# sayands/sgaligner

Measured on AMD Instinct MI355X. Metric: subscan-pairs/sec (fwd+bwd) + node-match Hits@1 vs reference, higher is better.
Workload: dtype f32 (fp32 operands and fp32 accumulation throughout; the anchors x negatives loss sweeps multiply them as three exact bf16 planes, six bf16 MFMAs per product...

## Files before the change

sgaligner_amd/csrc/sweep3.hip:

```cpp
#include <type_traits>

#include "loss_math.h"
#include "s3_layout.h"

namespace {

__device__ __forceinline__ void split3_pair(float v0, float v1, unsigned& h, unsigned& m, unsigned& l) {
    const bf16x2 H = __builtin_convertvector(f32x2{v0, v1}, bf16x2);
    const unsigned hu = __builtin_bit_cast(unsigned, H);
#ifdef S3_SPLIT_DOT2
    unsigned c0 = 0x0000BF80u, c1 = 0xBF800000u;
    asm("" : "+s"(c0), "+s"(c1));
    const bf16x2 n0 = __builtin_bit_cast(bf16x2, c0), n1 = __builtin_bit_cast(bf16x2, c1);
    const float r0 = __builtin_amdgcn_fdot2_f32_bf16(H, n0, v0, false);
    const float r1 = __builtin_amdgcn_fdot2_f32_bf16(H, n1, v1, false);
#else
    const float r0 = v0 - __builtin_bit_cast(float, hu << 16);
    const float r1 = v1 - __builtin_bit_cast(float, hu & 0xffff0000u);
#endif
    const bf16x2 Mi = __builtin_convertvector(f32x2{r0, r1}, bf16x2);
    const unsigned mu = __builtin_bit_cast(unsigned, Mi);
#ifdef S3_SPLIT_DOT2
    const float s0 = __builtin_amdgcn_fdot2_f32_bf16(Mi, n0, r0, false);
    const float s1 = __builtin_amdgcn_fdot2_f32_bf16(Mi, n1, r1, false);
// ... 74 lines not shown
    __syncthreads();
    if (threadIdx.x < 32) {
        const int r = threadIdx.x;
        if (r < nvalid) {
            double a = 0.0;
            for (int c = 0; c < S3_DREAL; ++c) a += (double)zbar[c] * (double)tile[r * S3_DP + c];
            tile[r * S3_DP + S3_DREAL] = (float)(a + (double)stat[S3_DP]);
            tile[r * S3_DP + S3_DREAL + 1] = 1.f;
        }
    }
    __syncthreads();
    unsigned* out = reinterpret_cast<unsigned*>(Zb + (size_t)blockIdx.x * S3_BLOCK);
    for (int e = threadIdx.x; e < 3 * 2 * 64 * 4; e += 256) {
        const int p = e & 3, st = (e >> 2) & 63, jh = (e >> 8) & 1, q = e >> 9;
        const int g = st >> 4, i = (st & 15) ^ (12 * (g & 1));
        const int row = 8 * (i >> 2) + 4 * jh + (i & 3), col = 32 * q + 8 * g + 2 * p;
        unsigned h, m, l;
        split3_pair(tile[row * S3_DP + col], tile[row * S3_DP + col + 1], h, m, l);
        out[e] = h; out[S3_PLANE / 4 + e] = m; out[2 * S3_PLANE / 4 + e] = l;
    }
    for (int e = threadIdx.x; e < 2 * 64 * 4; e += 256) {
        const int p = e & 3, st = (e >> 2) & 63, jh = (e >> 8) & 1;
        const int g = st >> 4, i = (st & 15) ^ (12 * (g & 1));
        const int row = 8 * (i >> 2) + 4 * jh + (i & 3), col = 96 + 2 * p;
        unsigned h, m, l;
        split3_pair(tile[row * S3_DP + col], tile[row * S3_DP + col + 1], h, m, l);
        out[S3_TAIL / 4 + e] = g < 2 ? h : (g == 2 ? m : l);
    }
}


__global__ __launch_bounds__(256) void centre_tables_kernel(const float* __restrict__ Z, int R, const float* __restrict__ stat, float* __restrict__ Zc) {
    const int lane = threadIdx.x & 63, wpb = blockDim.x >> 6;
    for (int r = blockIdx.x * wpb + (threadIdx.x >> 6); r < R; r += gridDim.x * wpb) {
        const float* z = Z + (size_t)r * S3_DP;
        float* o = Zc + (size_t)r * S3_DP;
        double acc = 0.0;
        float v[2];
#pragma unroll
        for (int t = 0; t < 2; ++t) {
            const int d = lane + 64 * t;
            const float zb = d < S3_DREAL ? stat[d] : 0.f;
            v[t] = d < S3_DREAL ? z[d] - zb : 0.f;
            acc += (double)zb * (double)v[t];
        }
        acc = wave_sum_d(acc);
        o[lane] = v[0];
        const int d1 = lane + 64;
        if (d1 < S3_DP) o[d1] = d1 < S3_DREAL ? v[1] : (d1 == S3_DREAL ? (float)(acc + (double)stat[S3_DP]) : (d1 == S3_DREAL + 1 ? 1.f : 0.f));
    }
}

#ifdef S3_DBG_TIMING
__device__ unsigned long long g_s3_dbg[16];
#define S3_T(i) { const unsigned long long t_ = __builtin_readcyclecounter(); tacc[i] += t_ - tprev; tprev = t_; }
#else
#define S3_T(i)
#endif
struct TSeg { int blk0, jt_lo, jt_hi, old0, lo, hi, fam; };
struct TGroup { int own0, nown, own_old0, own_blk0, blk0, nsplit, nseg; TSeg seg[2]; };
struct TArgs {
    int M; const unsigned char* Zb[4]; int perm[4]; int ngroups; TGroup grp[4];
    float k0, k1, it0, it1, ka;
    const float* beta;
    double* sums;
    const double* gs;
    float* dZ[4];
    double* gamma;
};

#ifndef S3_PAIR
#define S3_PAIR 1
#endif
template <int M, int PER> struct S3PairGaps {
    int slot[M][40];
    constexpr S3PairGaps() : slot{} {
        for (int p = 0; p < M; ++p) {
            int n = 0;
            for (int P = 0; P < 40; ++P) {
                const bool copy = p < M - 1 && P % (20 / PER) == 1 && P / (20 / PER) < 2 * PER;
                slot[p][P] = (P >= 3 && !copy) ? n++ : -1;
            }
        }
    }
};

template <int M, bool GRAD, int WV, int MG, bool GAM, bool LITE, bool FOLD>
__device__ __forceinline__ void sweep3_body(const TArgs& a, const int g) {
    static_assert(!LITE || !GRAD, "LITE: the forward sums only");
    static_assert(!FOLD || (GRAD && WV == 4), "FOLD: the one-wave-per-SIMD gradient sweep only");
    constexpr int NCT = 7;
    constexpr int WAVES = WV, THREADS = WAVES * 64;
    constexpr int OWN = WV * 16;
    constexpr int NCH = LITE ? S3_NCH - S3_PLANE / 1024 : S3_NCH;
    constexpr int KMAX = (NCH + WAVES - 1) / WAVES;
    constexpr int BUF = M * S3_BLOCK;
    constexpr bool PIPE = WV == 4;
#ifndef S3_OWN_IN_S
#define S3_OWN_IN_S 1
#endif
    constexpr bool OWN_IN_S = GRAD && PIPE && S3_OWN_IN_S;
#ifndef S3_SPREAD
#define S3_SPREAD 1
#endif
    constexpr bool SPREAD = OWN_IN_S && S3_SPREAD && !FOLD;
    constexpr bool PAIR_FITS = !(!GRAD && WV == 8 && M == 3 && !LITE);
    constexpr bool PAIR_DEFAULT = !(GRAD && M == 2) && !(!GRAD && M == 4 && !LITE);
    constexpr bool PAIR = PAIR_FITS && (S3_PAIR == 2 || (S3_PAIR == 1 && PAIR_DEFAULT));
    extern __shared__ __attribute__((aligned(16))) unsigned char lds3[];

    const int tid = threadIdx.x, lane = tid & 63, wave = tid >> 6, g4 = lane >> 4, l15 = lane & 15;
    const TGroup& grp = a.grp[g];
    const int wg_in_grp = (int)blockIdx.x - grp.blk0;
    const int nsplit = grp.nsplit, n_ob = (grp.nown + OWN - 1) / OWN, n_units = n_ob * nsplit;
    const int unit = (wg_in_grp & 7) * ((n_units + 7) >> 3) + (wg_in_grp >> 3);
    if ((wg_in_grp >> 3) >= ((n_units + 7) >> 3) || unit >= n_units) return;
    const int split = unit / n_ob;
    const int own0 = grp.own0 + (unit - split * n_ob) * OWN;
    const int own_end = grp.own0 + grp.nown;
    const int wrow0 = own0 + wave * 16;
#ifdef S3_DBG_TIMING
    unsigned long long tacc[8] = {0, 0, 0, 0, 0, 0, 0, 0}, tprev = __builtin_readcyclecounter();
#endif

    u32x4 opl[M][3][3], otl[M][2];
    float beta[M];
    const bool iv = wrow0 + l15 < own_end;
    {
        const int my_i = wrow0 + l15;
        const int rel = (iv ? my_i : own0) - grp.own_old0;
        const int o = rel & 31, oi = 4 * (o >> 3) + (o & 3), ojh = (o >> 2) & 1;
        const size_t off = (size_t)(grp.own_blk0 + (rel >> 5)) * S3_BLOCK;
#pragma unroll
        for (int m = 0; m < M; ++m) {
            const unsigned char* base = a.Zb[m] + off;
#pragma unroll
            for (int p = 0; p < 3; ++p)
#pragma unroll
                for (int q = 0; q < 3; ++q) {
                    const int so = ((q * 2 + ojh) * 64 + s3_slot(g4, oi)) * 16;
                    opl[m][p][q] = iv ? *reinterpret_cast<const u32x4*>(base + p * S3_PLANE + so) : u32x4{0, 0, 0, 0};
                }
            u32x4 th = iv ? *reinterpret_cast<const u32x4*>(base + S3_TAIL + (ojh * 64 + s3_slot(0, oi)) * 16) : u32x4{0, 0, 0, 0};
            u32x4 tm = iv ? *reinterpret_cast<const u32x4*>(base + S3_TAIL + (ojh * 64 + s3_slot(2, oi)) * 16) : u32x4{0, 0, 0, 0};
            u32x4 tl = iv ? *reinterpret_cast<const u32x4*>(base + S3_TAIL + (ojh * 64 + s3_slot(3, oi)) * 16) : u32x4{0, 0, 0, 0};
            const float ksc = a.k1;
            auto rescale = [&](u32x4& ph, u32x4& pm, u32x4& pl) {
#pragma unroll
                for (int d = 0; d < 4; ++d) {
                    const float x0 = (__builtin_bit_cast(float, ph[d] << 16) + __builtin_bit_cast(float, pm[d] << 16)) + __builtin_bit_cast(float, pl[d] << 16);
                    const float x1 = (__builtin_bit_cast(float, ph[d] & 0xffff0000u) + __builtin_bit_cast(float, pm[d] & 0xffff0000u)) + __builtin_bit_cast(float, pl[d] & 0xffff0000u);
                    unsigned nh, nm, nl;
                    split3_pair(x0 * ksc, x1 * ksc, nh, nm, nl);
                    ph[d] = nh; pm[d] = nm; pl[d] = nl;
                }
            };
#pragma unroll
            for (int q = 0; q < 3; ++q) rescale(opl[m][0][q], opl[m][1][q], opl[m][2][q]);
            rescale(th, tm, tl);
            s3_own_tails(th, tm, tl, g4, otl[m]);
        }
// ... 42 lines not shown
        buf_off = (unsigned)(buf - lds3);
#pragma unroll
        for (int m = 0; m < M; ++m) {
            trot[m] = tile_off + crot[m]; brot[m] = buf_off + (unsigned)(m * S3_BLOCK) + crot[m];
            asm("" : "+s"(trot[m]), "+s"(brot[m]));
        }
    };
    auto issue_slots = [&](int f_lo, int f_hi) {
#ifdef S3_DBG_NODMA
        return;
#endif
#ifdef S3_DBG_DMA_WAVES
        unsigned dma_mask = S3_DBG_DMA_WAVES;
        asm volatile("" : "+s"(dma_mask));
        if (!((dma_mask >> wave_u) & 1u)) return;
#endif
#pragma unroll
        for (int f = f_lo; f < f_hi; ++f) {
            if (f >= M * KMAX) break;
            const int m = f / KMAX, k = f % KMAX;
            unsigned so, lo;
            if (LAST_ODD && k == KMAX - 1) { so = tile_off + clast[m]; lo = buf_off + (unsigned)(m * S3_BLOCK) + clast[m]; }
            else { so = trot[m] + (unsigned)(k * WAVES * 1024); lo = brot[m] + (unsigned)(k * WAVES * 1024); }
            __builtin_amdgcn_raw_ptr_buffer_load_lds(rs[m], (lds_ptr)lds3 + lo, 16, l16, so, 0, 0);
        }
    };
    auto issue = [&](int jt, unsigned char* buf) { set_tile(jt, buf); issue_slots(0, M * KMAX); };

    const int aoff = s3_slot(g4, l15) * 16;
    const int tr_io = 4 * g4 + (l15 >> 2), tr_cs = l15 & 3;
    const int tr_main = s3_slot(tr_cs >> 1, tr_io) * 16 + (tr_cs & 1) * 8;
    const int tr_tail = S3_TAIL + tr_io * 16 + (tr_cs & 1) * 8;
    const int tr_tail_l = S3_TAIL + (48 + (tr_io ^ 12)) * 16 + (tr_cs & 1) * 8;

#pragma unroll 1
    for (int sg = 0; sg < 2; ++sg) {
        if (sg >= grp.nseg) break;
        const TSeg seg = grp.seg[sg];
        set_seg(seg);
        float c0[M + 1], c1[M + 1];
#pragma unroll
        for (int m = 0; m <= M; ++m) {
            const int mo = m < M ? a.perm[m] : M;
            c0[m] = GRAD ? (float)(a.gs[mo * 8 + seg.fam * 2 + 0] * (double)a.it0) : 0.f;
            c1[m] = GRAD ? (float)(a.gs[mo * 8 + seg.fam * 2 + 1] * (double)a.it1) : 0.f;
        }
        const float ka = a.ka;
        double dsum[M + 1][2];
#pragma unroll
        for (int m = 0; m <= M; ++m) { dsum[m][0] = 0.0; dsum[m][1] = 0.0; }
        float pl0[LITE ? M + 1 : 1], pl1[LITE ? M + 1 : 1];
#pragma unroll
        for (int m = 0; m < (LITE ? M + 1 : 1); ++m) { pl0[m] = 0.f; pl1[m] = 0.f; }

        __syncthreads();
        if (seg.jt_lo + split < seg.jt_hi) issue(seg.jt_lo + split, lds3);
        int it = 0;
#pragma unroll 1
        for (int jt = seg.jt_lo + split; jt < seg.jt_hi; jt += nsplit, ++it) {
            unsigned char* buf = lds3 + (it & 1) * BUF;
            const int j0 = seg.old0 + 32 * jt;
            S3_T(5)
            __syncthreads();
            S3_T(0)
            const int next_jt = jt + nsplit < seg.jt_hi ? jt + nsplit : jt;
            unsigned char* next_buf = lds3 + ((it + 1) & 1) * BUF;
            set_tile(next_jt, next_buf);
            S3_T(1)
            if (GRAD) {
                const int vlo = max(seg.lo - j0, 0), vhi = min(seg.hi - j0, 32);
                if (vlo > 0 || vhi < 32) {
                    for (int x = tid; x < M * 32 * S3_ROWSLOTS; x += THREADS) {
                        const int pc = x % S3_ROWSLOTS, w = (x / S3_ROWSLOTS) % 32, m = x / (S3_ROWSLOTS * 32);
                        if (w >= vlo && w < vhi) continue;
                        const int wjh = (w >> 2) & 1, wi = 4 * (w >> 3) + (w & 3);
                        unsigned char* base = buf + m * S3_BLOCK;
                        if (pc < 36) {
                            const int pl = pc / 12, q = (pc % 12) >> 2, gq = pc & 3;
                            *reinterpret_cast<u32x4*>(base + pl * S3_PLANE + ((q * 2 + wjh) * 64 + s3_slot(gq, wi)) * 16) = u32x4{0, 0, 0, 0};
                        } else {
                            const int gq = pc - 36;
                            *reinterpret_cast<u32x4*>(base + S3_TAIL + (wjh * 64 + s3_slot(gq, wi)) * 16) = u32x4{0, 0, 0, 0};
                        }
                    }
                    __syncthreads();
                }
            }

            f32x4 sacc[M][2];
            float own[M][2][4];
            float cj[2][4];
            auto substep_wait = [&](int ss) {
                if (ss > 0) { __builtin_amdgcn_s_waitcnt(0xc07f); __builtin_amdgcn_sched_barrier(0); }
            };
            constexpr int NSET = (PIPE || PAIR) ? 2 : 1;
            u32x4 at[NSET], ap[NSET][3][3];
            auto ld_one = [&](int ss, int idx) {
                const int e = ss % NSET;
                const unsigned char* ar = buf + (SPREAD ? ss % M : ss >> 1) * S3_BLOCK + (SPREAD ? ss / M : ss & 1) * 1024 + aoff;
                if (idx < 1) at[e] = *reinterpret_cast<const u32x4*>(ar + S3_TAIL);
                else ap[e][2 - (idx - 1) / 3][(idx - 1) % 3] = *reinterpret_cast<const u32x4*>(ar + (2 - (idx - 1) / 3) * S3_PLANE + ((idx - 1) % 3) * 2048);
            };
            auto ld_set = [&](int ss) {
#pragma unroll
                for (int idx = 0; idx < 10; ++idx) if (!(LITE && idx >= 1 && idx <= 3)) ld_one(ss, idx);
            };
            if (PIPE) {
                ld_set(0);
                if (PAIR) ld_set(1);
                __builtin_amdgcn_s_waitcnt(0xc07f);
                __builtin_amdgcn_sched_barrier(0);
            }
            auto lgkm_wait = [&](int n) {
                if (n == 0) __builtin_amdgcn_s_waitcnt(0xc07f);
                else if (n == 6) __builtin_amdgcn_s_waitcnt(0xc67f);
                else if (n == 8) __builtin_amdgcn_s_waitcnt(0xc87f);
                else __builtin_amdgcn_s_waitcnt(0xce7f);
                __builtin_amdgcn_sched_barrier(0);
            };
            if constexpr (SPREAD && PAIR) {
                constexpr int NDS = 2 * M - 2, PER = (M * KMAX + NDS - 1) / NDS, CS = 20 / PER;
// ... 88 lines not shown
                        for (int mm = 0; mm < M; ++mm) sjt = fmaf(beta[mm], sacc[mm][hh][r], sjt);
                    } else if (k == 1) ce0 = fexp2(sjt * ka);
                    else if (k == 2) ce1 = fexp2(sjt);
                    else cj[hh][r] = c0[M] * ce0 + c1[M] * ce1;
                };
#pragma unroll
                for (int ss = 0; ss < 2 * M; ++ss) {
                    const int m = ss % M, jh = ss / M, e = ss % NSET, pa = ss & 1;
                    const int pm = ss > 0 ? (ss - 1) % M : 0, pjh = ss > 0 ? (ss - 1) / M : 0;
                    accp[pa][0] = f32x4{0.f, 0.f, 0.f, 0.f}; accp[pa][1] = f32x4{0.f, 0.f, 0.f, 0.f};
                    substep_wait(ss);
#pragma unroll
                    for (int x = 0; x < 20; ++x) {
                        if (x == 0) accp[pa][0] = mfma_b(at[e], otl[m][1], accp[pa][0]);
                        else if (x == 1) accp[pa][1] = mfma_b(at[e], otl[m][0], accp[pa][1]);
                        else accp[pa][x & 1] = mfma_b(ap[e][PA[(x - 2) / 3]][(x - 2) % 3], opl[m][PB[(x - 2) / 3]][(x - 2) % 3], accp[pa][x & 1]);
                        __builtin_amdgcn_sched_barrier(0);
                        if (ss + 1 < 2 * M && x < 10) ld_one(ss + 1, x);
                        if (ss < NDS && (x % 3) == 1 && (x / 3) < PER) issue_slots(ss * PER + (x / 3), ss * PER + (x / 3) + 1);
                        if (ss > 0) {
                            if (x == 0) { sacc[pm][pjh][0] = accp[pa ^ 1][0][0] + accp[pa ^ 1][1][0]; sacc[pm][pjh][1] = accp[pa ^ 1][0][1] + accp[pa ^ 1][1][1]; }
                            if (x == 2) { sacc[pm][pjh][2] = accp[pa ^ 1][0][2] + accp[pa ^ 1][1][2]; sacc[pm][pjh][3] = accp[pa ^ 1][0][3] + accp[pa ^ 1][1][3]; }
                            if (pm < MG) {
                                constexpr int G0[4] = {3, 8, 12, 16}, G1[4] = {5, 9, 14, 17}, G2[4] = {6, 11, 15, 18};
#pragma unroll
                                for (int r = 0; r < 4; ++r) {
                                    if (x == G0[r]) own_step(pm, pjh, r, 0);
                                    if (x == G1[r]) own_step(pm, pjh, r, 1);
                                    if (x == G2[r]) own_step(pm, pjh, r, 2);
                                }
                            }
                        }
                        if (ss >= NDS) {
                            const int q = (x == 19 ? 5 : (x % 3) == 1 && x <= 13 ? x / 3 : -1);
                            if (q >= 0) {
                                const int qq = (ss - NDS) * 6 + q, r = qq / 3, k = qq % 3;
                                if (k == 0) { if (r > 0) cj_step(0, r - 1, 3); cj_step(0, r, 0); }
                                else cj_step(0, r, k);
                            }
                        }
                        __builtin_amdgcn_sched_barrier(0);
                    }
                }
#pragma unroll
                for (int r = 0; r < 4; ++r) sacc[M - 1][1][r] = accp[(2 * M - 1) & 1][0][r] + accp[(2 * M - 1) & 1][1][r];
                cj_step(0, 3, 3);
            } else if constexpr (PAIR) {
                constexpr int NDS = GRAD ? (2 * M - 2) : 2 * M, PER = (M * KMAX + NDS - 1) / NDS, CS = 20 / PER;
                static_assert(!PIPE || (2 * PER * CS <= 40 && (NDS / 2) * 2 * PER >= M * KMAX), "paired S stream: the copies' gaps");
                constexpr int PA[6] = {2, 1, 1, 0, 0, 0}, PB[6] = {0, 1, 0, 2, 1, 0};
#pragma unroll
                for (int m = 0; m < M; ++m) {
                    const bool nxt = m + 1 < M;
                    if (!PIPE) { ld_set(2 * m); ld_set(2 * m + 1); }
                    if (PIPE && m > 0) lgkm_wait(6);
                    f32x4 accq[2] = {f32x4{0.f, 0.f, 0.f, 0.f}, f32x4{0.f, 0.f, 0.f, 0.f}};
                    float ownt[2] = {0.f, 0.f};
#pragma unroll
                    for (int P = 0; P < 40; ++P) {
                        const int x = P >> 1, s = P & 1;
                        const bool skip = LITE && x >= 2 && (PA[(x - 2) / 3] == 2 || PB[(x - 2) / 3] == 2 || (PA[(x - 2) / 3] == 1 && PB[(x - 2) / 3] == 1));
                        if (skip) {}
                        else if (x == 0) accq[s] = mfma_b(at[s], otl[m][1], accq[s]);
                        else if (x == 1) accq[s] = mfma_b(at[s], otl[m][0], accq[s]);
                        else accq[s] = mfma_b(ap[s][PA[(x - 2) / 3]][(x - 2) % 3], opl[m][PB[(x - 2) / 3]][(x - 2) % 3], accq[s]);
                        if (PIPE) {
                            __builtin_amdgcn_sched_barrier(0);
                            if (nxt) {
                                const int sn = 2 * m + 2 + s;
                                if (P >= 2 && P < 4) ld_one(sn, 0);
                                else if (P >= 4 && P < 10) { if (!LITE) ld_one(sn, 1 + (P - 4) / 2); }
                                else if (P >= 16 && P < 22) ld_one(sn, 4 + (P - 16) / 2);
                                else if (P >= 34) ld_one(sn, 7 + (P - 34) / 2);
                            }
                            if (m < NDS / 2 && (P % CS) == 1 && P / CS < 2 * PER) issue_slots(m * 2 * PER + P / CS, m * 2 * PER + P / CS + 1);
                            if (OWN_IN_S && m > 0 && m - 1 < MG && P >= 22 && P < 38) {
                                const int r8 = (P - 22) >> 1;
                                const float sv = sacc[m - 1][r8 >> 2][r8 & 3];
                                if (((P - 22) & 1) == 0) {
                                    ownt[0] = fexp2(sv * ka);
                                    ownt[1] = fexp2(sv);
                                } else {
                                    own[m - 1][r8 >> 2][r8 & 3] = fmaf(c0[m - 1], ownt[0], c1[m - 1] * ownt[1]);
                                }
                            }
                            if (m > 0 && P == 21) lgkm_wait(nxt ? (LITE ? 8 : 14) : 0);
                            __builtin_amdgcn_sched_barrier(0);
                        } else if (P == 1 && m < NDS / 2) {
                            issue_slots(2 * m * PER, (2 * m + 2) * PER);
                        }
                    }
#pragma unroll
                    for (int r = 0; r < 4; ++r) { sacc[m][0][r] = accq[0][r]; sacc[m][1][r] = accq[1][r]; }
                }
            } else {
#pragma unroll
            for (int ss = 0; ss < 2 * M; ++ss) {
                const int m = ss >> 1, jh = ss & 1, e = ss % NSET;
                if (!PIPE) ld_set(ss);
                if (PIPE) substep_wait(ss);
                constexpr int NDS = GRAD ? (2 * M - 2) : 2 * M, PER = (M * KMAX + NDS - 1) / NDS;
                f32x4 acc2[2] = {f32x4{0.f, 0.f, 0.f, 0.f}, f32x4{0.f, 0.f, 0.f, 0.f}};
                float ownt[2] = {0.f, 0.f};
                constexpr int PA[6] = {2, 1, 1, 0, 0, 0}, PB[6] = {0, 1, 0, 2, 1, 0};
#pragma unroll
                for (int x = 0; x < 20; ++x) {
                    const bool skip = LITE && x >= 2 && (PA[(x - 2) / 3] == 2 || PB[(x - 2) / 3] == 2 || (PA[(x - 2) / 3] == 1 && PB[(x - 2) / 3] == 1));
                    if (skip) {}
                    else if (x == 0) acc2[0] = mfma_b(at[e], otl[m][1], acc2[0]);
                    else if (x == 1) acc2[1] = mfma_b(at[e], otl[m][0], acc2[1]);
                    else acc2[x & 1] = mfma_b(ap[e][PA[(x - 2) / 3]][(x - 2) % 3], opl[m][PB[(x - 2) / 3]][(x - 2) % 3], acc2[x & 1]);
                    if (PIPE) {
                        __builtin_amdgcn_sched_barrier(0);
                        if (ss + 1 < 2 * M && x < 10 && !(LITE && x >= 1 && x <= 3)) ld_one(ss + 1, x);
                        if (ss < NDS && (x % 3) == 1 && (x / 3) < PER) issue_slots(ss * PER + (x / 3), ss * PER + (x / 3) + 1);
                        if (OWN_IN_S && m > 0 && m - 1 < MG && x >= 11 && x < 19) {
                            const int r = (x - 11) >> 1;
                            const float sv = sacc[m - 1][jh][r];
                            if (((x - 11) & 1) == 0) {
                                ownt[0] = fexp2(sv * ka);
                                ownt[1] = fexp2(sv);
                            } else {
                                own[m - 1][jh][r] = fmaf(c0[m - 1], ownt[0], c1[m - 1] * ownt[1]);
                            }
                        }
                        __builtin_amdgcn_sched_barrier(0);
                    } else if (x == 1 && ss < NDS) {
                        issue_slots(ss * PER, (ss + 1) * PER);
                    }
                }
#pragma unroll
                for (int r = 0; r < 4; ++r) sacc[m][jh][r] = acc2[0][r] + acc2[1][r];
            }
            }

            S3_T(2)
            if (!GRAD) {
                float p0[M + 1], p1[M + 1];
#pragma unroll
                for (int m = 0; m <= M; ++m) { p0[m] = LITE ? pl0[LITE ? m : 0] : 0.f; p1[m] = LITE ? pl1[LITE ? m : 0] : 0.f; }
                auto sums_tile = [&](auto masked_c) {
                    constexpr bool MASKED = decltype(masked_c)::value;
#pragma unroll
                    for (int jh = 0; jh < 2; ++jh)
#pragma unroll
                        for (int r = 0; r < 4; ++r) {
                            const int row = j0 + 8 * g4 + 4 * jh + r;
                            const float okf = (!MASKED || (iv && row >= seg.lo && row < seg.hi)) ? 1.f : 0.f;
                            float sj = 0.f;
#pragma unroll
                            for (int m = 0; m < M; ++m) {
                                const float sv = sacc[m][jh][r];
                                sj = fmaf(beta[m], sv, sj);
                                p0[m] = MASKED ? fmaf(okf, fexp2(sv * ka), p0[m]) : p0[m] + fexp2(sv * ka);
                                p1[m] = MASKED ? fmaf(okf, fexp2(sv), p1[m]) : p1[m] + fexp2(sv);
                            }
                            p0[M] = MASKED ? fmaf(okf, fexp2(sj * ka), p0[M]) : p0[M] + fexp2(sj * ka);
                            p1[M] = MASKED ? fmaf(okf, fexp2(sj), p1[M]) : p1[M] + fexp2(sj);
                        }
                };
                if (j0 >= seg.lo && j0 + 32 <= seg.hi && own0 + OWN <= own_end) sums_tile(std::false_type{}); else sums_tile(std::true_type{});
                if (!LITE || (it & 3) == 3) {
#pragma unroll
                    for (int m = 0; m <= M; ++m) { dsum[m][0] += (double)p0[m]; dsum[m][1] += (double)p1[m]; }
#pragma unroll
                    for (int m = 0; m < (LITE ? M + 1 : 1); ++m) { pl0[m] = 0.f; pl1[m] = 0.f; }
                } else {
#pragma unroll
                    for (int m = 0; m < (LITE ? M + 1 : 1); ++m) { pl0[m] = p0[m]; pl1[m] = p1[m]; }
                }
            } else {
                constexpr int BD = PIPE ? 4 : 1;
                u32x4 bp[BD][3];
                auto ld_b = [&](int k) {
                    const int m = k / NCT, ct = k % NCT, par = k % BD;
                    const unsigned char* pb = buf + m * S3_BLOCK;
#pragma unroll
                    for (int p = 0; p < 3; ++p) {
                        const unsigned char* ph = ct < 6 ? pb + p * S3_PLANE + tr_main + (ct >> 1) * 2048 + (ct & 1) * 512
                                                         : pb + (p == 2 ? tr_tail_l : tr_tail + (p == 1 ? 512 : 0));
                        const u32x2 x0 = tr_read16(ph), x1 = tr_read16(ph + 1024);
                        bp[par][p] = u32x4{x0[0], x0[1], x1[0], x1[1]};
                    }
                };
                constexpr int OWN_LAST0 = (SPREAD && PAIR) ? (M > 2 ? M - 2 : 1) : M - 1;
                auto own_late = [&](int mm) {
#pragma unroll
                    for (int r = 0; r < 4; ++r) {
                        const float sv = sacc[mm][1][r];
                        own[mm][1][r] = fmaf(c0[mm], fexp2(sv * ka), c1[mm] * fexp2(sv));
                    }
                };
                auto own_last = [&]() {
#pragma unroll
                    for (int mm = OWN_LAST0; mm < M; ++mm) if (mm < MG) own_late(mm);
                };
                if (SPREAD && PAIR && M == 2) own_late(0);
#pragma unroll
                for (int m = SPREAD ? M : OWN_IN_S ? M - 1 : 0; m < MG; ++m)
#pragma unroll
                    for (int jh = 0; jh < 2; ++jh)
#pragma unroll
                        for (int r = 0; r < 4; ++r) {
                            const float sv = sacc[m][jh][r];
#ifdef S3_DBG_NOEPI
                            own[m][jh][r] = sv;
#else
                            own[m][jh][r] = fmaf(c0[m], fexp2(sv * ka), c1[m] * fexp2(sv));
#endif
                        }
#pragma unroll
                for (int jh = SPREAD ? 1 : 0; jh < 2; ++jh)
#pragma unroll
                    for (int r = 0; r < 4; ++r) {
                        float sj = 0.f;
#pragma unroll
                        for (int m = 0; m < M; ++m) sj = fmaf(beta[m], sacc[m][jh][r], sj);
#ifdef S3_DBG_NOEPI
                        cj[jh][r] = sj;
#else
                        cj[jh][r] = c0[M] * fexp2(sj * ka) + c1[M] * fexp2(sj);
#endif
                    }
// ... 44 lines not shown
                        if (m > 0) planes(m);
#pragma unroll
                        for (int ct = 0; ct < NCT; ++ct) {
                            ld_b(NCT * m + ct);
#pragma unroll
                            for (int i = 0; i < 5; ++i) step_small(m, ct, 0, i);
                            gacc[GRAD ? m : 0][ct] = mfma_b(ch[m & 1], bp[0][0], gacc[GRAD ? m : 0][ct]);
                        }
                    }
                } else {
                    __builtin_amdgcn_sched_barrier(0);
                    ld_b(0); ld_b(1);
                    __builtin_amdgcn_sched_barrier(0);
#pragma unroll
                    for (int g4i = 0; g4i < 4 * MG; ++g4i) {
                        const int m = g4i >> 2, ct0 = (g4i & 3) * 2, n = (g4i & 3) == 3 ? 1 : 2, k0_ = NCT * m + ct0;
                        if (SPREAD && g4i == 0 && OWN_LAST0 < MG && M > 1) own_last();
                        if ((g4i & 3) == 0 && m + 1 < MG) planes(m + 1);
                        if (GAM && !FOLD && g4i == (MG > 1 ? 4 : 0)) gamma_acc();
                        if (FOLD && g4i >= 2) fold_group(g4i - 2);
                        const int kn = k0_ + n;
                        const int nn = kn >= NCT * MG ? 0 : ((kn % NCT) == 6 ? 1 : 2);
#pragma unroll
                        for (int j = 0; j < nn; ++j) ld_b(kn + j);
                        if (n == 2) {
#pragma unroll
                            for (int i = 0; i < 5; ++i) { step_small(m, ct0, k0_ % BD, i); step_small(m, ct0 + 1, (k0_ + 1) % BD, i); }
                            gacc[GRAD ? m : 0][ct0] = mfma_b(ch[m & 1], bp[k0_ % BD][0], gacc[GRAD ? m : 0][ct0]);
                            gacc[GRAD ? m : 0][ct0 + 1] = mfma_b(ch[m & 1], bp[(k0_ + 1) % BD][0], gacc[GRAD ? m : 0][ct0 + 1]);
                        } else {
                            step_small(m, ct0, k0_ % BD, 0);
                            gacc[GRAD ? m : 0][ct0] = mfma_b(ch[m & 1], bp[k0_ % BD][0], gacc[GRAD ? m : 0][ct0]);
#pragma unroll
                            for (int i = 1; i < 5; ++i) step_small(m, ct0, k0_ % BD, i);
                        }
                        if (FOLD) {
                            if (n == 2) { if (nn == 2) sgb_seq<0, 12, 12, true>(); else if (nn == 1) sgb_seq<0, 12, 6, true>(); else sgb_seq<0, 12, 0, true>(); }
                            else { if (nn == 2) sgb_seq<0, 6, 12, false>(); else if (nn == 1) sgb_seq<0, 6, 6, false>(); else sgb_seq<0, 6, 0, false>(); }
                        } else {
#pragma unroll
                        for (int x = 0; x < 6 * n; ++x) {
                            __builtin_amdgcn_sched_group_barrier(0x008, 1, 0);
                            if (x < 6 * nn) __builtin_amdgcn_sched_group_barrier(0x100, 1, 0);
                            if (n == 2 || x < 2) __builtin_amdgcn_sched_group_barrier(0x002, 2, 0);
                        }
                        }
                        if ((g4i & 3) == 3) __builtin_amdgcn_sched_barrier(0);
                    }
                    if (FOLD) { fold_group(4 * MG - 2); fold_group(4 * MG - 1); }
                }
                S3_T(4)
            }
        }
        if (!GRAD) {
#pragma unroll
            for (int m = 0; m <= M; ++m)
#pragma unroll
                for (int tt = 0; tt < 2; ++tt) {
                    if (LITE) dsum[m][tt] += (double)(tt ? pl1[LITE ? m : 0] : pl0[LITE ? m : 0]);
                    const double v = wave_sum_d(dsum[m][tt]);
                    if (lane == 0 && v != 0.0) atomicAdd(a.sums + (M + 1) * 8 * (1 + my_slot()) + m * 8 + seg.fam * 2 + tt, v);
                }
        }
    }
#ifdef S3_DBG_TIMING
    if (lane == 0) for (int i = 0; i < 8; ++i) atomicAdd(&g_s3_dbg[(GRAD ? 8 : 0) + i], tacc[i]);
#endif
    if (GRAD) {
#pragma unroll
        for (int m = 0; m < MG; ++m) {
            float* dz = a.dZ[m];
#pragma unroll
            for (int ct = 0; ct < NCT; ++ct) if (!FOLD) gacc[GRAD ? m : 0][ct] += gsm[(GRAD && !FOLD) ? m : 0][ct];
#pragma unroll
            for (int ct = 0; ct < NCT; ++ct) {
                const int d = ct * 16 + l15;
                if (d < S3_DREAL || d == S3_DREAL + 1) {
#pragma unroll
                    for (int r = 0; r < 4; ++r) {
                        const int i = wrow0 + 4 * g4 + r;
                        if (i < own_end) atomicAdd(dz + (size_t)i * S3_DP + d, gacc[GRAD ? m : 0][ct][r]);
                    }
                }
            }
        }
        if (GAM && g < 2) {
#pragma unroll
            for (int m = 0; m < M; ++m) {
                const float v = wave_sum(gam[m]) / a.k1;
                if (lane == 0 && v != 0.f) atomicAdd(a.gamma + M * (1 + my_slot()) + a.perm[m], (double)v);
            }
        }
    }
}

template <int M, bool GRAD, int WV, int MG = M, bool GAM = true, bool LITE = false, bool FOLD = false>
__global__ __launch_bounds__(WV * 64, WV == 8 ? 2 : 1) void sweep3_kernel(TArgs a) {
    int g = 0;
#pragma unroll
    for (int i = 1; i < 4; ++i) if (i < a.ngroups && (int)blockIdx.x >= a.grp[i].blk0) g = i;
#ifndef S3_GAM_ALL
    if constexpr (GRAD && GAM) {
        if (g >= 2) { sweep3_body<M, GRAD, WV, MG, false, LITE, FOLD>(a, g); return; }
    }
#endif
    sweep3_body<M, GRAD, WV, MG, GAM, LITE, FOLD>(a, g);
}

struct SProd { const float* S; int ld, tn, own_seg, own0, nown, oth_seg, oth0, noth, blk0, nsplit; };
struct SArgs { const unsigned char* Zb; float* dZ; const float* zero; int A, nbA, n; SProd p[4]; };

__global__ __launch_bounds__(256, 2) void stash3_kernel(SArgs a) {
    constexpr int NCT = 7, WAVES = 4, RW = 2, OWN = WAVES * RW * 16;
    constexpr int KMAX = (S3_NCH + WAVES - 1) / WAVES;
    extern __shared__ __attribute__((aligned(16))) unsigned char lds3[];
    const int tid = threadIdx.x, lane = tid & 63, wave = tid >> 6, g4 = lane >> 4, l15 = lane & 15;
    int pi = 0;
#pragma unroll
    for (int i = 1; i < 4; ++i) if (i < a.n && (int)blockIdx.x >= a.p[i].blk0) pi = i;
    const SProd& P = a.p[pi];
    const float* const PS = P.S;
    const float* const zero_word = a.zero;
    const int Pld = P.ld, Ptn = P.tn, Pnown = P.nown, Poth0 = P.oth0, Pnoth = P.noth;
    const int w_in = (int)blockIdx.x - P.blk0;
    const int n_ob = (P.nown + OWN - 1) / OWN;
    if (w_in >= n_ob * P.nsplit) return;
    const int split = w_in / n_ob, ob = w_in - split * n_ob;
    const int orow0 = ob * OWN + wave * (RW * 16) + l15;
    const int t_lo = P.oth0 >> 5, t_hi = (P.oth0 + P.noth + 31) >> 5;
    const int per = (t_hi - t_lo + P.nsplit - 1) / P.nsplit;
    const int jt0 = t_lo + split * per, jt1 = min(t_hi, jt0 + per);
    if (jt0 >= jt1) return;
    const int oblk0 = P.oth_seg ? a.nbA : 0;

    const int wave_u = __builtin_amdgcn_readfirstlane(wave);
    unsigned l16 = threadIdx.x;
    asm volatile("" : "+v"(l16));
    l16 = (l16 & 63u) * 16u;
    auto issue = [&](int blk, unsigned char* buf) {
        const unsigned long long tb = sreg64(reinterpret_cast<unsigned long long>(a.Zb) + (unsigned long long)blk * S3_BLOCK);
#pragma unroll
        for (int k = 0; k < KMAX; ++k) {
            int c = wave_u + k * WAVES;
            if ((k + 1) * WAVES > S3_NCH) c = c >= S3_NCH ? c - WAVES : c;
            __builtin_amdgcn_global_load_lds((const __attribute__((address_space(1))) void*)(reinterpret_cast<const unsigned char*>(tb + (unsigned)(c * 1024)) + l16),
                                             (__attribute__((address_space(3))) void*)(buf + c * 1024), 16, 0, 0);
        }
    };
    auto load_c = [&](int jt, int rs, float (&c)[8]) {
        const int orow = orow0 + 16 * rs;
        const bool ov = orow < Pnown;
        const int r0 = 32 * jt + 8 * g4 - Poth0;
        if (!Ptn && (Pld & 3) == 0 && (Poth0 & 3) == 0 && ov && r0 >= 0 && r0 + 8 <= Pnoth) {
            const f32x4* q = reinterpret_cast<const f32x4*>(PS + (size_t)orow * Pld + r0);
            const f32x4 u = q[0], v = q[1];
            c[0] = u[0]; c[1] = u[1]; c[2] = u[2]; c[3] = u[3]; c[4] = v[0]; c[5] = v[1]; c[6] = v[2]; c[7] = v[3];
        } else {
            const float* base = PS + (Ptn ? (size_t)orow : (size_t)orow * Pld);
// ... 120 lines not shown
        const TSeg X1f0{bx1, jl, jh, ox1, ox1 + a_lo, ox1 + a_hi, 0}, X2f3{bx2, jl, jh, ox2, ox2 + a_lo, ox2 + a_hi, 3};
        const TSeg X1f1{bx1, jl, jh, ox1, ox1 + a_lo, ox1 + a_hi, 1}, X2f2{bx2, jl, jh, ox2, ox2 + a_lo, ox2 + a_hi, 2};
        add(on1, J1, on1, bn1, X1f0, X2f3);
        add(on2, J2, on2, bn2, X1f1, X2f2);
    }
    a.ngroups = g;
    for (int i = 0; i < g; ++i)
        for (int sg = 0; sg < a.grp[i].nseg; ++sg)
            if ((long long)a.grp[i].seg[sg].jt_hi * S3_BLOCK >= (1LL << 32)) {
                sga_set_error("%s: a segment of %d 32-row blocks exceeds the 4 GiB a copy descriptor spans", who, a.grp[i].seg[sg].jt_hi);
                return SGA_ERR_ARG;
            }
    int nwg = 0;
    for (int i = 0; i < g; ++i) {
        TGroup& G = a.grp[i];
        int steps = 0;
        for (int sg = 0; sg < G.nseg; ++sg) steps += G.seg[sg].jt_hi - G.seg[sg].jt_lo;
        const long n_ob_g = (G.nown + own_rows - 1) / own_rows;
        const long want = (long)steps * n_ob_g / (12L * sga_num_cus());
        const int unit_steps = want < 160 ? 160 : want > 640 ? 640 : (int)want;
        int nsp = (steps + unit_steps - 1) / unit_steps;
        if (nsp > steps) nsp = steps;
        if (nsp < 1) nsp = 1;
        G.nsplit = nsp;
        G.blk0 = nwg;
        nwg += (((G.nown + own_rows - 1) / own_rows) * nsp + 7) / 8 * 8;
    }
    return -nwg;
}

#ifndef S3_WV_SUMS
#define S3_WV_SUMS 8
#endif
#ifndef S3_WV_GRAD3
#define S3_WV_GRAD3 4
#endif
#ifndef S3_WV_GRAD2
#define S3_WV_GRAD2 4
#endif
template <int M, bool GRAD> constexpr int s3_wv() { return M == 4 ? 4 : GRAD ? (M == 3 ? S3_WV_GRAD3 : S3_WV_GRAD2) : S3_WV_SUMS; }

template <int M, bool GRAD, int MG = M, bool GAM = true, bool LITE = false, bool FOLD = false>
void launch_t(const TArgs& a, int nwg, hipStream_t s) {
    constexpr int WV = s3_wv<M, GRAD>();
    const size_t lds = (size_t)2 * M * S3_BLOCK;
    auto k = sweep3_kernel<M, GRAD, WV, MG, GAM, LITE, FOLD>;
    hipFuncSetAttribute(reinterpret_cast<const void*>(k), hipFuncAttributeMaxDynamicSharedMemorySize, (int)lds);
    hipLaunchKernelGGL(k, dim3(nwg), dim3(WV * 64), lds, s, a);
}

}

#ifdef S3_DBG_TIMING
extern "C" int sga_dbg_sweep3(unsigned long long* host16) {
    if (hipMemcpyFromSymbol(host16, HIP_SYMBOL(g_s3_dbg), sizeof(g_s3_dbg)) != hipSuccess) return 1;
    static unsigned long long z[16];
    return hipMemcpyToSymbol(HIP_SYMBOL(g_s3_dbg), z, sizeof(z)) != hipSuccess;
}
#endif

extern "C" size_t sga_loss_split3_bytes(int A, int J1, int J2) {
    const TLayout L = make_tlayout(A, J1, J2);
    return (size_t)(2 * L.nbA + L.nb1 + L.nb2 + 1) * S3_BLOCK + S3_STAT_BYTES + (size_t)S3_CS_BLOCKS * S3_DP * sizeof(double);
}

extern "C" int sga_loss_split3_tables(const float* Z, int A, int J1, int J2, void* Zb, float* Zc, void* stream) {
    SGA_CHECK_ARG(A >= 0 && J1 >= 0 && J2 >= 0, "sga_loss_split3_tables: bad sizes");
    const TLayout L = make_tlayout(A, J1, J2);
    const int nb = 2 * L.nbA + L.nb1 + L.nb2;
    if (nb == 0) return SGA_OK;
    SGA_CHECK_ARG(Z && Zb, "sga_loss_split3_tables: null pointer");
    hipStream_t s = static_cast<hipStream_t>(stream);
    unsigned char* tail = static_cast<unsigned char*>(Zb) + (size_t)nb * S3_BLOCK;
    if (hipMemsetAsync(tail, 0, S3_BLOCK + S3_STAT_BYTES, s) != hipSuccess) { sga_set_error("sga_loss_split3_tables: memset failed"); return SGA_ERR_HIP; }
    float* stat = reinterpret_cast<float*>(tail + S3_BLOCK);
    double* part = reinterpret_cast<double*>(tail + S3_BLOCK + S3_STAT_BYTES);
    const int R = 2 * A + J1 + J2;
    const int ncs = R < 64 * S3_CS_BLOCKS ? (R + 63) / 64 : S3_CS_BLOCKS;
    hipLaunchKernelGGL(split3_colsum_kernel, dim3(ncs), dim3(128), 0, s, Z, R, part);
    hipLaunchKernelGGL(split3_stats_kernel, dim3(1), dim3(128), 0, s, part, ncs, R, stat);
    hipLaunchKernelGGL(split3_tables_kernel, dim3(nb), dim3(256), 0, s, Z, A, J1, J2, static_cast<unsigned char*>(Zb), stat, Zc);
    SGA_CHECK_LAUNCH("sga_loss_split3_tables");
    return SGA_OK;
}

extern "C" size_t sga_loss_centre_bytes(void) { return S3_STAT_BYTES + (size_t)S3_CS_BLOCKS * S3_DP * sizeof(double); }

extern "C" int sga_loss_centre_tables(const float* Z, int A, int J1, int J2, float* Zc, void* stat_ws, void* stream) {
    SGA_CHECK_ARG(A >= 0 && J1 >= 0 && J2 >= 0, "sga_loss_centre_tables: bad sizes");
    const int R = 2 * A + J1 + J2;
    SGA_CHECK_ARG(stat_ws, "sga_loss_centre_tables: null statistics workspace");
    hipStream_t s = static_cast<hipStream_t>(stream);
    if (hipMemsetAsync(stat_ws, 0, S3_STAT_BYTES, s) != hipSuccess) { sga_set_error("sga_loss_centre_tables: memset failed"); return SGA_ERR_HIP; }
    if (R == 0) return SGA_OK;
    SGA_CHECK_ARG(Z && Zc, "sga_loss_centre_tables: null pointer");
    float* stat = static_cast<float*>(stat_ws);
    double* part = reinterpret_cast<double*>(static_cast<unsigned char*>(stat_ws) + S3_STAT_BYTES);
    const int ncs = R < 64 * S3_CS_BLOCKS ? (R + 63) / 64 : S3_CS_BLOCKS;
    hipLaunchKernelGGL(split3_colsum_kernel, dim3(ncs), dim3(128), 0, s, Z, R, part);
    hipLaunchKernelGGL(split3_stats_kernel, dim3(1), dim3(128), 0, s, part, ncs, R, stat);
    int grid = (R + 3) / 4;
    if (grid > 8 * sga_num_cus()) grid = 8 * sga_num_cus();
    hipLaunchKernelGGL(centre_tables_kernel, dim3(grid), dim3(256), 0, s, Z, R, stat, Zc);
    SGA_CHECK_LAUNCH("sga_loss_centre_tables");
    return SGA_OK;
}

__global__ void scatter_tangent_kernel(const float* __restrict__ dZ, const float* __restrict__ Z, const float* __restrict__ nrm,
                                       const int* __restrict__ idx, int R, int D, const float* __restrict__ stat, float* __restrict__ dE) {
// ... 147 lines not shown
```

Measured before the change: 998.0.

## De-phase half the waves in the LITE forward sums sweep to overlap epilogue

In the forward LITE M=3 sums sweep with 8 waves, the upper half of the waves now runs a DEFER variant. That variant issues all its LDS slot loads right after the barrier and delays the exp/sum epilogue of the previous tile until the next tile's MFMA loop begins. The intent is to offset the MFMA and transcendental phases across waves so that the matrix and VALU pipes overlap, instead of every wave hitting the epilogue at once. It also adds an unconditional vmcnt wait before each barrier, and it keeps a copy of the accumulators across iterations, which raises register pressure. The debug timing buffer grows to hold the new variant's counters.

```diff
diff --git a/sgaligner_amd/csrc/sweep3.hip b/sgaligner_amd/csrc/sweep3.hip
--- a/sgaligner_amd/csrc/sweep3.hip
+++ b/sgaligner_amd/csrc/sweep3.hip
@@ -150,7 +150,7 @@
 }
 
 #ifdef S3_DBG_TIMING
-__device__ unsigned long long g_s3_dbg[16];
+__device__ unsigned long long g_s3_dbg[24];
 #define S3_T(i) { const unsigned long long t_ = __builtin_readcyclecounter(); tacc[i] += t_ - tprev; tprev = t_; }
 #else
 #define S3_T(i)
@@ -170,6 +170,20 @@
 #ifndef S3_PAIR
 #define S3_PAIR 1
 #endif
+#ifndef S3_PHASE
+#define S3_PHASE 1
+#endif
+#ifndef S3_PHASE_ODD
+#define S3_PHASE_ODD 0
+#endif
+#ifndef S3_PHASE_PRIO
+#define S3_PHASE_PRIO 0
+#endif
+template <int M, bool GRAD, int WV, bool LITE> constexpr bool s3_phase() {
+    constexpr bool FITS = !GRAD && WV == 8 && !(M == 3 && !LITE);
+    constexpr bool DEFAULT = M == 3 && LITE;
+    return FITS && (S3_PHASE == 2 || (S3_PHASE == 1 && DEFAULT));
+}
 template <int M, int PER> struct S3PairGaps {
     int slot[M][40];
     constexpr S3PairGaps() : slot{} {
@@ -183,7 +197,7 @@
     }
 };
 
-template <int M, bool GRAD, int WV, int MG, bool GAM, bool LITE, bool FOLD>
+template <int M, bool GRAD, int WV, int MG, bool GAM, bool LITE, bool FOLD, bool DEFER = false>
 __device__ __forceinline__ void sweep3_body(const TArgs& a, const int g) {
     static_assert(!LITE || !GRAD, "LITE: the forward sums only");
     static_assert(!FOLD || (GRAD && WV == 4), "FOLD: the one-wave-per-SIMD gradient sweep only");
@@ -205,6 +219,7 @@
     constexpr bool PAIR_FITS = !(!GRAD && WV == 8 && M == 3 && !LITE);
     constexpr bool PAIR_DEFAULT = !(GRAD && M == 2) && !(!GRAD && M == 4 && !LITE);
     constexpr bool PAIR = PAIR_FITS && (S3_PAIR == 2 || (S3_PAIR == 1 && PAIR_DEFAULT));
+    static_assert(!DEFER || s3_phase<M, GRAD, WV, LITE>(), "DEFER: the de-phased forward sums only (S3_PHASE)");
     extern __shared__ __attribute__((aligned(16))) unsigned char lds3[];
 
     const int tid = threadIdx.x, lane = tid & 63, wave = tid >> 6, g4 = lane >> 4, l15 = lane & 15;
@@ -353,6 +368,45 @@
         float pl0[LITE ? M + 1 : 1], pl1[LITE ? M + 1 : 1];
 #pragma unroll
         for (int m = 0; m < (LITE ? M + 1 : 1); ++m) { pl0[m] = 0.f; pl1[m] = 0.f; }
+        auto sums_epi = [&](const f32x4 (&sa)[M][2], const int ej0, const int eit) {
+            float p0[M + 1], p1[M + 1];
+#pragma unroll
+            for (int m = 0; m <= M; ++m) { p0[m] = LITE ? pl0[LITE ? m : 0] : 0.f; p1[m] = LITE ? pl1[LITE ? m : 0] : 0.f; }
+            auto sums_tile = [&](auto masked_c) {
+                constexpr bool MASKED = decltype(masked_c)::value;
+#pragma unroll
+                for (int jh = 0; jh < 2; ++jh)
+#pragma unroll
+                    for (int r = 0; r < 4; ++r) {
+                        const int row = ej0 + 8 * g4 + 4 * jh + r;
+                        const float okf = (!MASKED || (iv && row >= seg.lo && row < seg.hi)) ? 1.f : 0.f;
+                        float sj = 0.f;
+#pragma unroll
+                        for (int m = 0; m < M; ++m) {
+                            const float sv = sa[m][jh][r];
+                            sj = fmaf(beta[m], sv, sj);
+                            p0[m] = MASKED ? fmaf(okf, fexp2(sv * ka), p0[m]) : p0[m] + fexp2(sv * ka);
+                            p1[m] = MASKED ? fmaf(okf, fexp2(sv), p1[m]) : p1[m] + fexp2(sv);
+                        }
+                        p0[M] = MASKED ? fmaf(okf, fexp2(sj * ka), p0[M]) : p0[M] + fexp2(sj * ka);
+                        p1[M] = MASKED ? fmaf(okf, fexp2(sj), p1[M]) : p1[M] + fexp2(sj);
+                    }
+            };
+            if (ej0 >= seg.lo && ej0 + 32 <= seg.hi && own0 + OWN <= own_end) sums_tile(std::false_type{}); else sums_tile(std::true_type{});
+            if (!LITE || (eit & 3) == 3) {
+#pragma unroll
+                for (int m = 0; m <= M; ++m) { dsum[m][0] += (double)p0[m]; dsum[m][1] += (double)p1[m]; }
+#pragma unroll
+                for (int m = 0; m < (LITE ? M + 1 : 1); ++m) { pl0[m] = 0.f; pl1[m] = 0.f; }
+            } else {
+#pragma unroll
+                for (int m = 0; m < (LITE ? M + 1 : 1); ++m) { pl0[m] = p0[m]; pl1[m] = p1[m]; }
+            }
+        };
+        f32x4 csacc[M][2];
+        int cj0 = 0;
+#pragma unroll
+        for (int m = 0; m < M; ++m) { csacc[m][0] = f32x4{0.f, 0.f, 0.f, 0.f}; csacc[m][1] = f32x4{0.f, 0.f, 0.f, 0.f}; }
 
         __syncthreads();
         if (seg.jt_lo + split < seg.jt_hi) issue(seg.jt_lo + split, lds3);
@@ -362,12 +416,14 @@
             unsigned char* buf = lds3 + (it & 1) * BUF;
             const int j0 = seg.old0 + 32 * jt;
             S3_T(5)
+            if (S3_PHASE) __builtin_amdgcn_s_waitcnt(0x0f70);
             __syncthreads();
             S3_T(0)
             const int next_jt = jt + nsplit < seg.jt_hi ? jt + nsplit : jt;
             unsigned char* next_buf = lds3 + ((it + 1) & 1) * BUF;
             set_tile(next_jt, next_buf);
             S3_T(1)
+            if (DEFER) { issue_slots(0, M * KMAX); S3_T(1) }
             if (GRAD) {
                 const int vlo = max(seg.lo - j0, 0), vhi = min(seg.hi - j0, 32);
                 if (vlo > 0 || vhi < 32) {
@@ -562,6 +618,7 @@
 #pragma unroll
                 for (int m = 0; m < M; ++m) {
                     const bool nxt = m + 1 < M;
+                    if (DEFER && m == 0 && it > 0) { sums_epi(csacc, cj0, it - 1); S3_T(3) }
                     if (!PIPE) { ld_set(2 * m); ld_set(2 * m + 1); }
                     if (PIPE && m > 0) lgkm_wait(6);
                     f32x4 accq[2] = {f32x4{0.f, 0.f, 0.f, 0.f}, f32x4{0.f, 0.f, 0.f, 0.f}};
@@ -596,7 +653,7 @@
                             }
                             if (m > 0 && P == 21) lgkm_wait(nxt ? (LITE ? 8 : 14) : 0);
                             __builtin_amdgcn_sched_barrier(0);
-                        } else if (P == 1 && m < NDS / 2) {
+                        } else if (P == 1 && m < NDS / 2 && !DEFER) {
                             issue_slots(2 * m * PER, (2 * m + 2) * PER);
                         }
                     }
@@ -607,6 +664,7 @@
 #pragma unroll
             for (int ss = 0; ss < 2 * M; ++ss) {
                 const int m = ss >> 1, jh = ss & 1, e = ss % NSET;
+                if (DEFER && ss == 0 && it > 0) { sums_epi(csacc, cj0, it - 1); S3_T(3) }
                 if (!PIPE) ld_set(ss);
                 if (PIPE) substep_wait(ss);
                 constexpr int NDS = GRAD ? (2 * M - 2) : 2 * M, PER = (M * KMAX + NDS - 1) / NDS;
@@ -635,7 +693,7 @@
                             }
                         }
                         __builtin_amdgcn_sched_barrier(0);
-                    } else if (x == 1 && ss < NDS) {
+                    } else if (x == 1 && ss < NDS && !DEFER) {
                         issue_slots(ss * PER, (ss + 1) * PER);
                     }
                 }
@@ -646,6 +704,12 @@
 
             S3_T(2)
             if (!GRAD) {
+                if (DEFER) {
+#pragma unroll
+                    for (int m = 0; m < M; ++m) { csacc[m][0] = sacc[m][0]; csacc[m][1] = sacc[m][1]; }
+                    cj0 = j0;
+                }
+                if (!DEFER) {
                 float p0[M + 1], p1[M + 1];
 #pragma unroll
                 for (int m = 0; m <= M; ++m) { p0[m] = LITE ? pl0[LITE ? m : 0] : 0.f; p1[m] = LITE ? pl1[LITE ? m : 0] : 0.f; }
@@ -679,6 +743,8 @@
 #pragma unroll
                     for (int m = 0; m < (LITE ? M + 1 : 1); ++m) { pl0[m] = p0[m]; pl1[m] = p1[m]; }
                 }
+                }
+                S3_T(3)
             } else {
                 constexpr int BD = PIPE ? 4 : 1;
                 u32x4 bp[BD][3];
@@ -829,6 +895,7 @@
                 S3_T(4)
             }
         }
+        if (DEFER && it > 0) { sums_epi(csacc, cj0, it - 1); S3_T(3) }
         if (!GRAD) {
 #pragma unroll
             for (int m = 0; m <= M; ++m)
@@ -841,7 +908,7 @@
         }
     }
 #ifdef S3_DBG_TIMING
-    if (lane == 0) for (int i = 0; i < 8; ++i) atomicAdd(&g_s3_dbg[(GRAD ? 8 : 0) + i], tacc[i]);
+    if (lane == 0) for (int i = 0; i < 8; ++i) atomicAdd(&g_s3_dbg[(GRAD ? 8 : DEFER ? 16 : 0) + i], tacc[i]);
 #endif
     if (GRAD) {
 #pragma unroll
@@ -881,6 +948,14 @@
         if (g >= 2) { sweep3_body<M, GRAD, WV, MG, false, LITE, FOLD>(a, g); return; }
     }
 #endif
+    if constexpr (s3_phase<M, GRAD, WV, LITE>()) {
+        const int wave_u = __builtin_amdgcn_readfirstlane((int)(threadIdx.x >> 6));
+        if (S3_PHASE_ODD ? (wave_u & 1) != 0 : wave_u >= WV / 2) {
+            if (S3_PHASE_PRIO) __builtin_amdgcn_s_setprio(1);
+            sweep3_body<M, GRAD, WV, MG, GAM, LITE, FOLD, true>(a, g);
+            return;
+        }
+    }
     sweep3_body<M, GRAD, WV, MG, GAM, LITE, FOLD>(a, g);
 }
 
@@ -1107,9 +1182,9 @@
 }
 
 #ifdef S3_DBG_TIMING
-extern "C" int sga_dbg_sweep3(unsigned long long* host16) {
-    if (hipMemcpyFromSymbol(host16, HIP_SYMBOL(g_s3_dbg), sizeof(g_s3_dbg)) != hipSuccess) return 1;
-    static unsigned long long z[16];
+extern "C" int sga_dbg_sweep3(unsigned long long* host24) {
+    if (hipMemcpyFromSymbol(host24, HIP_SYMBOL(g_s3_dbg), sizeof(g_s3_dbg)) != hipSuccess) return 1;
+    static unsigned long long z[24];
     return hipMemcpyToSymbol(HIP_SYMBOL(g_s3_dbg), z, sizeof(z)) != hipSuccess;
 }
 #endif
```

Result: no change. 1003, median of 6 (+0.5%).
